# AnishDelft/ModelCompression

Measured on AMD Instinct MI355X. Metric: images/sec (fwd+bwd, 416x416), higher is better.
Workload: dtype fp16

## Files before the change

### include/mcamd.h

```cpp
#ifndef MCAMD_H
#define MCAMD_H

#include <stddef.h>
#include <stdint.h>

#ifdef __cplusplus
extern "C" {
#endif

#define MCAMD_OK 0
#define MCAMD_EINVAL (-1)
#define MCAMD_ELAUNCH (-2)
#define MCAMD_EWORKSPACE (-3)

int mcamd_version(void);
void mcamd_reload_config(void);
const char* mcamd_arch(void);
const char* mcamd_last_error(void);

typedef struct mcamd_conv_geom {
    int32_t B, H, W;
    int32_t ksize;
    int32_t cin;
    int32_t cout;
// ... 160 lines not shown
    int32_t ch_lo, C;
} mcamd_dgrad_sums;
int32_t mcamd_conv_dgrad_sums_rows(const mcamd_conv_geom* g, int32_t concurrent);
int mcamd_conv_dgrad_sums(const mcamd_conv_geom* g, const void* dy, int32_t dy_ld, int32_t dy_choff,
                          const void* wp_dgrad, const mcamd_conv_epilogue* epi, const mcamd_dgrad_sums* sums, void* stream);

size_t mcamd_conv_wgrad_workspace_bytes(const mcamd_conv_geom* g);
int mcamd_conv_wgrad(const mcamd_conv_geom* g, const void* x, const void* dy, int32_t dy_ld,
                     int32_t dy_choff, const float* mask_oihw, const mcamd_chan_map* map,
                     float grad_scale, float* dw_oihw, float* dbias, void* workspace,
                     size_t workspace_bytes, void* stream);

#define MCAMD_WGRAD_GENERIC 0
#define MCAMD_WGRAD_STEM 1
#define MCAMD_WGRAD_WIN 2
#define MCAMD_WGRAD_NINE 3
#define MCAMD_WGRAD_NINE_WIDE 4
#define MCAMD_WFIN_ROW 0
#define MCAMD_WFIN_VEC 1
#define MCAMD_WFIN_GENERIC 2
#define MCAMD_WGRAD_PLAN_INFO_N 13
int mcamd_conv_wgrad_plan_info(const mcamd_conv_geom* g, int32_t has_cmap, int32_t out[MCAMD_WGRAD_PLAN_INFO_N]);
int32_t mcamd_wgrad_generic_instances(int32_t* out, int32_t cap);

int mcamd_bn_coeffs(const float* stats, int32_t stats_rows, int32_t stats_ld, int32_t C, int64_t count,
                    const float* gamma, const float* beta, float* running_mean, float* running_var,
                    float momentum, float eps, int32_t training,
                    float* scale, float* shift, float* save_mean, float* save_invstd,
                    const int32_t* chan_perm, void* stream);

int mcamd_bn_coeffs_ex(const float* stats, int32_t stats_rows, int32_t stats_ld, int32_t C, int64_t count,
                       const float* gamma, const float* beta, float* running_mean, float* running_var,
                       float momentum, float eps, int32_t training,
                       float* scale, float* shift, float* save_mean, float* save_invstd,
                       const int32_t* chan_perm, int32_t ones_channel, void* stream);

#define MCAMD_DST_PLAIN 0
#define MCAMD_DST_POOL 1
#define MCAMD_DST_REORG 2
typedef struct mcamd_act_desc {
    int32_t B, H, W, C;
    const void* y; int32_t y_ld, y_choff;
    const float* scale; const float* shift;
    float slope;
    int32_t mode;
    void* dst; int32_t dst_ld, dst_choff;
// ... 328 lines not shown
```

### modelcompression_amd/_lib.py

```python
import ctypes as C
import os

_HERE = os.path.dirname(os.path.abspath(__file__))
LIB_PATH = os.path.join(_HERE, "libmcamd.so")


class McamdError(RuntimeError):
    pass


class ConvGeom(C.Structure):
    _fields_ = [("B", C.c_int32), ("H", C.c_int32), ("W", C.c_int32), ("ksize", C.c_int32),
                ("cin", C.c_int32), ("cout", C.c_int32), ("x_ld", C.c_int32), ("x_choff", C.c_int32),
                ("stem", C.c_int32), ("pad", C.c_int32), ("x_wrap", C.c_int32), ("x_f8", C.c_int32), ("x_f8_wexp", C.c_int32)]


class ConvEpilogue(C.Structure):
    _fields_ = [("mode", C.c_int32), ("y_ld", C.c_int32), ("y_choff", C.c_int32),
                ("y", C.c_void_p), ("bias", C.c_void_p), ("stats", C.c_void_p),
                ("stats_rows", C.c_int32), ("stats_ld", C.c_int32),
                ("scale", C.c_void_p), ("shift", C.c_void_p), ("slope", C.c_float), ("overflow", C.c_void_p),
                ("dst_mode", C.c_int32), ("y2", C.c_void_p), ("y2_ld", C.c_int32), ("y2_choff", C.c_int32),
                ("concurrent", C.c_int32)]

# ... 127 lines not shown


class WzSeg(C.Structure):
    _fields_ = [("w", C.c_void_p), ("mask", C.c_void_p), ("n", C.c_int64), ("word0", C.c_int64), ("val0", C.c_int64),
                ("kept", C.c_int64), ("cout", C.c_int32), ("kind", C.c_int32), ("exp0", C.c_int32), ("dense", C.c_int32),
                ("block0", C.c_int32), ("shift0", C.c_int32)]


class HzSeg(C.Structure):
    _fields_ = [("sym0", C.c_int64), ("nsym", C.c_int64), ("nbits", C.c_int64), ("word0", C.c_int64), ("chunk0", C.c_int64),
                ("popc_bits", C.c_int64), ("block0", C.c_int32), ("A", C.c_int32)]


class WsSeg(C.Structure):
    _fields_ = [("w", C.c_void_p), ("mask", C.c_void_p), ("codes", C.c_void_p), ("n", C.c_int64), ("part0", C.c_int64),
                ("K", C.c_int32), ("cb0", C.c_int32), ("slab0", C.c_int32), ("reserved", C.c_int32)]


EPI_RAW_F16, EPI_NCHW_F32, EPI_PAD_F16, EPI_RAW_F32 = 0, 1, 2, 3
DST_PLAIN, DST_POOL, DST_REORG = 0, 1, 2
WGRAD_GENERIC, WGRAD_STEM, WGRAD_WIN, WGRAD_NINE, WGRAD_NINE_WIDE = 0, 1, 2, 3, 4
WFIN_ROW, WFIN_VEC, WFIN_GENERIC = 0, 1, 2
WGRAD_PLAN_INFO_N = 13
STEM_PLAN_FWD, STEM_PLAN_FWD_PLANES, STEM_PLAN_STATS, STEM_PLAN_GRAM, STEM_PLAN_BWD = 0, 1, 2, 3, 4
STEM_PLAN_INFO_N = 20
WZ_FP32, WZ_FP16, WZ_FP8, WZ_CODE, WZ_W4 = 0, 1, 2, 4, 5
WZ_F_BN, WZ_F_BITS = 1, 2
WZ_BLOCK_WORDS = 64
HZ_MAXLEN, HZ_CHUNK, HZ_GROUP = 12, 1024, 64
WS_SLAB = 4096

_P, _I32, _I64, _F, _SZ = C.c_void_p, C.c_int32, C.c_int64, C.c_float, C.c_size_t
SIGNATURES = {
    "mcamd_version": (C.c_int, []),
    "mcamd_arch": (C.c_char_p, []),
    "mcamd_last_error": (C.c_char_p, []),
    "mcamd_reload_config": (None, []),
    "mcamd_conv_stats_rows": (_I32, [C.POINTER(ConvGeom)]),
    "mcamd_conv_stats_rows_mode": (_I32, [C.POINTER(ConvGeom), _I32]),
    "mcamd_conv_fwd_f8_ok": (_I32, [C.POINTER(ConvGeom)]),
    "mcamd_conv_tile_info": (C.c_int, [C.POINTER(ConvGeom), _I32, C.POINTER(_I32)]),
    "mcamd_conv_route_info": (C.c_int, [C.POINTER(ConvGeom), _I32, _I32, _I32, _I32, C.POINTER(_I32)]),
    "mcamd_packed_elems_fwd": (_I64, [C.POINTER(ConvGeom)]),
    "mcamd_packed_elems_dgrad": (_I64, [C.POINTER(ConvGeom)]),
    "mcamd_pack_weights": (C.c_int, [C.POINTER(ConvGeom), _P, _P, C.POINTER(ChanMap), _P, _P, _P]),
    "mcamd_pack_weights_many": (C.c_int, [_P, _I32, _I64, _P]),
# ... 28 lines not shown
    "mcamd_conv_fwd_q8_sparse24_ok": (_I32, [C.POINTER(ConvGeom)]),
    "mcamd_q8_sparse24_elems": (C.c_int, [C.POINTER(ConvGeom), C.POINTER(_I64)]),
    "mcamd_pack_q8_sparse24": (C.c_int, [C.POINTER(ConvGeom), _P, _P, _P, _P, _P, _P]),
    "mcamd_conv_fwd_q8_sparse24": (C.c_int, [C.POINTER(ConvGeom), _P, _P, _P, _P, C.POINTER(ConvEpilogue), _I32, _I32, _P]),
    "mcamd_conv_fwd_q8_w4_ok": (_I32, [C.POINTER(ConvGeom)]),
    "mcamd_q8_w4_elems": (C.c_int, [C.POINTER(ConvGeom), C.POINTER(_I64)]),
    "mcamd_pack_q8_w4": (C.c_int, [C.POINTER(ConvGeom), _P, _P, _P, _P, _P, _P]),
    "mcamd_unpack_q8_w4": (C.c_int, [C.POINTER(ConvGeom), _P, _P, _P, _P]),
    "mcamd_conv_fwd_q8_w4": (C.c_int, [C.POINTER(ConvGeom), _P, _P, _P, _P, C.POINTER(ConvEpilogue), _I32, _I32, _P]),
    "mcamd_conv_fwd_q8_w4_info": (C.c_int, [C.POINTER(ConvGeom), C.POINTER(_I32)]),
    "mcamd_conv_fwd_q8_w4_raw": (C.c_int, [C.POINTER(ConvGeom), _P, _P, _P, _P, C.POINTER(ConvEpilogue), _P]),
    "mcamd_fakequant_q8_w4": (C.c_int, [C.POINTER(ConvGeom), _P, _P, _P, _P, _P]),
    "mcamd_cast_q8": (C.c_int, [_P, _I64, _I32, _I32, _I32, _P, _I32, _I32, _P]),
    "mcamd_conv_fwd_q8_stats_rows": (_I32, [C.POINTER(ConvGeom)]),
    "mcamd_fakequant_q8": (C.c_int, [C.POINTER(ConvGeom), _P, _P, _P, _P, _P]),
    "mcamd_cast_q8_train": (C.c_int, [_P, _I64, _I32, _I32, _I32, _P, _I32, _I32, _P]),
    "mcamd_conv_dgrad": (C.c_int, [C.POINTER(ConvGeom), _P, _I32, _I32, _P, C.POINTER(ConvEpilogue), _P]),
    "mcamd_conv_dgrad_sums_rows": (_I32, [C.POINTER(ConvGeom), _I32]),
    "mcamd_conv_dgrad_sums": (C.c_int, [C.POINTER(ConvGeom), _P, _I32, _I32, _P, C.POINTER(ConvEpilogue), C.POINTER(DgradSums), _P]),
    "mcamd_conv_wgrad_workspace_bytes": (_SZ, [C.POINTER(ConvGeom)]),
    "mcamd_conv_wgrad": (C.c_int, [C.POINTER(ConvGeom), _P, _P, _I32, _I32, _P, C.POINTER(ChanMap), _F, _P, _P, _P, _SZ, _P]),
    "mcamd_conv_wgrad_plan_info": (C.c_int, [C.POINTER(ConvGeom), _I32, C.POINTER(_I32)]),
    "mcamd_wgrad_generic_instances": (_I32, [C.POINTER(_I32), _I32]),
    "mcamd_bn_coeffs": (C.c_int, [_P, _I32, _I32, _I32, _I64, _P, _P, _P, _P, _F, _F, _I32, _P, _P, _P, _P, _P, _P]),
    "mcamd_bn_coeffs_ex": (C.c_int, [_P, _I32, _I32, _I32, _I64, _P, _P, _P, _P, _F, _F, _I32, _P, _P, _P, _P, _P, _I32, _P]),
    "mcamd_fold_weights": (C.c_int, [C.POINTER(FoldDesc), _P, _P]),
    "mcamd_fold_weights_many": (C.c_int, [_P, _I32, _I64, _P]),
    "mcamd_unfold_wgrad": (C.c_int, [C.POINTER(FoldDesc), _P, _P, _P, _P, _I32, _P]),
    "mcamd_bn_act_fwd": (C.c_int, [C.POINTER(ActDesc), _P]),
    "mcamd_bn_act_fwd_instance": (C.c_int, [C.POINTER(ActDesc), C.POINTER(ActInstance)]),
    "mcamd_bn_act_conv1x1_ok": (_I32, [C.POINTER(ActDesc), C.POINTER(ConvGeom)]),
    "mcamd_bn_act_conv1x1_stats_rows": (_I32, [C.POINTER(ActDesc), C.POINTER(ConvGeom)]),
    "mcamd_bn_act_conv1x1_fwd": (C.c_int, [C.POINTER(ActDesc), C.POINTER(ConvGeom), _P, C.POINTER(ConvEpilogue), _P]),
    "mcamd_bn_act_bwd_workspace_bytes": (_SZ, [C.POINTER(ActBwdDesc)]),
    "mcamd_bn_act_bwd": (C.c_int, [C.POINTER(ActBwdDesc), _P, _SZ, _P]),
    "mcamd_stem_block_workspace_bytes": (_SZ, []),
    "mcamd_stem_block_fwd": (C.c_int, [C.POINTER(StemBlockDesc), _P, _SZ, _P]),
    "mcamd_stem_block_bwd": (C.c_int, [C.POINTER(StemBlockDesc), _P, _SZ, _P]),
    "mcamd_stem_block_stats_rows": (_I32, [C.POINTER(StemBlockDesc)]),
    "mcamd_stem_block_stats": (C.c_int, [C.POINTER(StemBlockDesc), _P, _I32, _I32, _P]),
    "mcamd_stem_block_plan_info": (C.c_int, [C.POINTER(StemBlockDesc), C.POINTER(_I32)]),
    "mcamd_nchw_f32_to_nhwc4_split": (C.c_int, [_P, _I32, _I32, _I32, _P, _P, _P]),
    "mcamd_pack_stem_split": (C.c_int, [_P, _P, _I32, _P, _P, _P]),
    "mcamd_nchw_f32_to_padded_nhwc_f16": (C.c_int, [_P, _I32, _I32, _I32, _I32, _F, _P, _I32, _I32, _P, _P]),
    "mcamd_nchw_f32_to_padded_nhwc_f16_pad": (C.c_int, [_P, _I32, _I32, _I32, _I32, _F, _P, _I32, _I32, _I32, _P, _P]),
    "mcamd_nchw_f32_to_padded_nhwc_f16_split": (C.c_int, [_P, _I32, _I32, _I32, _I32, _P, _I32, _I32, _I32, _P]),
# ... 91 lines not shown
```

### modelcompression_amd/build.py

```python
import os
import subprocess
import sys
from concurrent.futures import ThreadPoolExecutor

HERE = os.path.dirname(os.path.abspath(__file__))
CSRC = os.path.join(HERE, "csrc")
OUT = os.path.join(HERE, "libmcamd.so")
HIPCC = os.environ.get("HIPCC", "/opt/rocm/bin/hipcc")
ARCH = "gfx950"
COMMON = ["--offload-arch=" + ARCH, "-O3", "-fPIC", "-std=c++17", "-Wall", "-Wno-unused-variable",
          "-fhip-fp32-correctly-rounded-divide-sqrt"]
SOURCES = {
    "api.hip": [],
    "conv_igemm.hip": [],
    "conv_igemm_pp.hip": [],
    "conv_sparse.hip": [],
    "conv_bsparse.hip": [],
    "conv_splitk.hip": [],
    "conv_q8.hip": [],
    "conv_q8_sparse.hip": [],
    "conv_q8_splitk.hip": [],
    "conv_q8_bsparse.hip": [],
    "conv_q8_w4.hip": [],
    "conv_stem.hip": [],
    "conv_stem_block.hip": [],
    "conv_stem_f32.hip": [],
    "conv_small.hip": [],
    "conv_win.hip": [],
    "conv_wres.hip": [],
    "conv_wgrad.hip": [],
    "conv_wgrad_stem.hip": [],
    "bn_act.hip": [],
    "bn_conv1x1.hip": [],
    "fold.hip": [],
    "plan.hip": [],
    "region_loss.hip": [],
    "distill_loss.hip": [],
    "prune.hip": ["-ffp-contract=off"],
    "augment.hip": ["-ffp-contract=off"],
    "detect.hip": ["-ffp-contract=off"],
    "voc_eval.hip": ["-ffp-contract=off"],
    "wpack.hip": ["-ffp-contract=off"],
    "wshare.hip": ["-ffp-contract=off"],
    "huff.hip": [],
}


def _stale(target, deps):
    if not os.path.exists(target):
        return True
    t = os.path.getmtime(target)
    return any(os.path.getmtime(d) > t for d in deps)


# ... 33 lines not shown
```

### modelcompression_amd/csrc/api.hip

```cpp
#include <stdarg.h>
#include <stdlib.h>
#include <string.h>

#include <string>

#include "kernels.h"

static thread_local char g_err[512] = "";

void mcamd_set_error(const char* fmt, ...) {
    va_list ap;
    va_start(ap, fmt);
    vsnprintf(g_err, sizeof(g_err), fmt, ap);
    va_end(ap);
}

int g_mcamd_env_generation = 0;
int McamdEnvSlot::get(const char* name, int dflt) {
    const int g = __atomic_load_n(&g_mcamd_env_generation, __ATOMIC_ACQUIRE);
    if (gen != g) {
        const char* s = getenv(name);
        has = s && *s ? 1 : 0;
        val = has ? atoi(s) : 0;
        __atomic_store_n(&gen, g, __ATOMIC_RELEASE);
// ... 1284 lines not shown
    a.dy_off = dy_choff + a.dy_row_stride + dy_ld;
    a.dy_zero_off = dy_choff;
    a.H = g->H, a.W = g->W, a.HW = g->H * g->W;
    a.M = (int)M;
    a.cin_tap = cin_tap;
    a.ntaps = ntaps;
    a.ktot = ntaps * cin_tap;
    fill_taps(g->ksize, g->stem, a.x_row_stride, g->x_ld, a.tap_off);
    int rc = p.nine    ? mcamd_wgrad9_launch(a, p, g->W + pw_of(g), padded_pixels(g), st)
             : p.stemw == 1 ? mcamd_wgrad_stem_launch(a, p, st)
             : p.stemw == 2 ? mcamd_wgrad_win_launch(a, p, st)
                       : mcamd_wgrad_launch(a, p, st);
    if (rc) return rc;
    rc = mcamd_wgrad_finish_launch((const float*)workspace, p, a.ktot, cin_tap, g->stem, g->cout, g->cin, g->ksize,
                                   mask_oihw, 1.0f / grad_scale, dw_oihw, rmap, cmap, st);
    if (rc) return rc;
    if (dbias) {
        long long rows = padded_pixels(g);
        rc = mcamd_colsum_launch((const half_t*)dy, rows, dy_ld, dy_choff, g->cout, 1.0f / grad_scale, dbias, st, workspace,
                                 workspace_bytes);
    }
    return rc;
}
```

### modelcompression_amd/csrc/kernels.h

```cpp
#pragma once
#include "common.h"

struct DgradSums {
    float* slab;
    const half_t* act;
    const float* scale;
    const float* shift;
    const float* mean;
    const float* invstd;
    const float* y;
    int act_ld, act_choff, act_pw;
    int y_ld, y_choff;
    int ch_lo, C;
    int ld;
    float slope;
};
#define MCAMD_EPI_RAW_F16_SUMS 4

struct IgemmArgs {
    const half_t* x;
    const half_t* w;
    void* y;
    const float* bias;
    float* stats;
// ... 121 lines not shown
int mcamd_pack_q8_sparse24_launch(const float* w, const float* mask, void* wq, void* idx, void* wexp, int cout, int cin,
                                  int ntaps, hipStream_t st);
Q8Choice mcamd_q8_w4_choice(long long M, int N);
int mcamd_conv_q8_w4_launch(IgemmArgs& a, const void* gshift, const void* wexp, int y_f8, int y2_f8, hipStream_t st);
int mcamd_pack_q8_w4_launch(const float* w, const float* mask, void* codes, void* gshift, void* wexp, int cout, int cin, int ntaps,
                            hipStream_t st);
int mcamd_unpack_q8_w4_launch(const void* codes, const void* gshift, void* wq, int cout, int cin, int ntaps, hipStream_t st);
int mcamd_conv_q8_w4_raw_launch(IgemmArgs& a, const void* gshift, const void* wexp, hipStream_t st);
int mcamd_fakequant_q8_w4_launch(const void* codes, const void* gshift, const void* wexp, float* out, int cout, int cin, int ntaps,
                                 hipStream_t st);

WgradPlan mcamd_wgrad_plan(long long M, int cout, int cin_tap, int ntaps);
int mcamd_wgrad_launch(WgradArgs& a, const WgradPlan& p, hipStream_t st);
bool mcamd_wgrad_stem_ok(int stem, int cout, int W, long long M);
WgradPlan mcamd_wgrad_stem_plan(long long M);
int mcamd_wgrad_stem_launch(WgradArgs& a, const WgradPlan& p, hipStream_t st);
bool mcamd_wgrad_win_ok(int ksize, int stem, int cout, int cin_tap, int W, long long M);
WgradPlan mcamd_wgrad_win_plan(long long M, int cout);
int mcamd_wgrad_win_launch(WgradArgs& a, const WgradPlan& p, hipStream_t st);
bool mcamd_wgrad_use9(int ksize, int stem, int cout, int cin_tap, int W);
WgradPlan mcamd_wgrad_plan9(long long P, int cout, int cin_tap, int W, int pitch, int B);
int mcamd_wgrad9_launch(const WgradArgs& w, const WgradPlan& p, int pitch, long long P, hipStream_t st);
WgradFinish mcamd_wgrad_finish_pick(int nsplit, int stem, int Cin, int ksize, bool has_cmap);
int mcamd_wgrad_instances(int (*out)[4], int cap);
int mcamd_wgrad_finish_launch(const float* slab, const WgradPlan& p, int ktot, int cin_tap, int stem, int Cout, int Cin,
                              int ksize, const float* mask, float inv_scale, float* dw, const int* rmap, const int* cmap,
                              hipStream_t st);
int mcamd_colsum_launch(const half_t* dy, long long rows, int ld, int choff, int C, float inv_scale, float* out,
                        hipStream_t st, void* scratch, size_t scratch_bytes);

bool mcamd_win3x3_ok(int mode, bool stats, long long M, int n, int cin_tap, int ktot, int H, int W);
int mcamd_win3x3_launch(const IgemmArgs& a, hipStream_t st);
bool mcamd_small3x3_ok(long long M, int n, int cin_tap, int ktot);
int mcamd_small3x3_rows(long long M);
int mcamd_small3x3_launch(const IgemmArgs& a, int rows, hipStream_t st);
bool mcamd_small3x3_split_ok(long long M, int n, int cin_tap, int ktot, int wrap, int mode);
int mcamd_small3x3_split_launch(const IgemmArgs& a, int rows, hipStream_t st);

bool mcamd_bn_conv1x1_shape_ok(int P, int cout);
int mcamd_bn_conv1x1_launch(IgemmArgs& a, const float* py, int py_ld, int py_choff, int P, int rows, hipStream_t st);

bool mcamd_wres_ok(int ksize, int stem, int n, int cin_tap, int ktot, int B, int H, int W, int mode);
int mcamd_wres_rows(int n, int B, int H, int W);
int mcamd_wres_launch(IgemmArgs& a, int B, int rows, hipStream_t st);

bool mcamd_stem_direct_ok(int stem, int cout, int mode);
// ... 3 lines not shown
```

### modelcompression_amd/engine.py

```python
import contextlib
import math
import os
import time

import torch

from . import ops
from . import _lib as L
from ._lib import McamdError


class _T:
    __slots__ = ("buf", "ld", "choff", "C", "H", "W", "ps", "ps0")

    def __init__(self, buf, ld, choff, C, H, W, ps=0):
        self.buf, self.ld, self.choff, self.C, self.H, self.W, self.ps = buf, ld, choff, C, H, W, ps
        self.ps0 = ps


_LAYER_FIELDS = dict(
    index=0, li=0, conv=None, bn=None, slope=1.0, src=0, tin=None, cin=0, cout=0, cout_p=0, H=0, W=0, k=0, M=0, stem=0, pad=0,
    level=1, mode=0, out_id=None, out2_id=None, out_t=None, out2_t=None, is_last=False, train_ok=True, border=None,
    border_map=None, geom=None, geom_f=None, p_lo=0, p_hi=0,
    wp=None, wd=None, y=None, stats=None, scale=None, shift=None, mean=None, invstd=None, dy=None, gin=None, act_full=None,
    keep=None, perm=None, perm32=None, in_perm=None, g_rows=None, g_cols=None, n_act=0, geom_act=None, gather=False,
    fold=None, fold_cin=0, fold_aug=0, fold_consumers=None, ones_idx=-1, skip_dead=False, bn_width=0, waug=None, dwaug=None,
    fused_stem=False, fused_stem_eval=False, stem_shadow=False, stem_split=False, stem_f32=False, stem_ws=None, weff=None,
    sh_img=None, sh_img_lo=None, sh_geom=None, sh_wp=None, sh_wp_lo=None, sh_coef=None,
    f8=False, f8_wexp=ops.F8_WEXP_DEFAULT, f8_wexp_eff=ops.F8_WEXP_DEFAULT,
    form="dense", sk_slices=1, wsp=None, widx=None, bs_count=None, bs_list=None,
    geom_q8=None, q8_y=False, q8_y2=False, xq=None, _xq=None, _xq_key=None, wq=None, wqs=None, widx8=None, wexp=None,
    w4c=None, w4g=None, wexp4=None,
    y_f16=None, stats_f16=None, y_f32=None, stats_q8=None, w_q=None)


class _Layer:
    __slots__ = tuple(_LAYER_FIELDS)

    def __init__(self):
        for name, default in _LAYER_FIELDS.items():
            setattr(self, name, default)
        self.fold_consumers = []

    sp_on = property(lambda self: self.form == "sparse24")
    bs_on = property(lambda self: self.form == "bsparse")
    sk_on = property(lambda self: self.form == "splitk")
# ... 516 lines not shown
                budget = int((MIXED_BUDGET / PLAIN_BLOCK_ERR) ** 2)
                unsplittable = len(self.layers) - len(can) - (1 if self.stem else 0)
                plain = set(l.li for l in by_cost[:max(0, budget - unsplittable)])
            for lay in can:
                if lay.li not in plain:
                    lay.level = 3
        f32 = dict(dtype=torch.float32, device=dev)
        wbytes = 0

        def li_is_first(l):
            return l.li == 0
        for lay in self.layers:
            g = lay.geom
            wrap = 2 * lay.tin.ps if (self.act_planes == 2 and lay.li > 0) else 0
            lay.geom_f = g if lay.level == 1 else ops.geom(B, lay.H, lay.W, lay.k, lay.level * lay.cin, lay.cout,
                                                           lay.tin.ld, 0, 0, lay.pad, wrap)
            nf, _ = ops.packed_elems(lay.geom_f)
            if self.precise:
                lay.n_act, lay.geom_act = lay.cout, g
                self._set_geom_f(lay)
            _, nd = ops.packed_elems(g)
            lay.wp = torch.zeros(nf, dtype=ops.HALF, device=dev)
            lay.wd = torch.zeros(nd, dtype=ops.HALF, device=dev) if (nd and lay.li > 0) else None
            wbytes = max(wbytes, ops.wgrad_workspace_bytes(g))
            lay.cout_p = ops.round_up(lay.cout, 32)
            lay.fused_stem = bool(lay.stem and lay.bn is not None and lay.mode == L.DST_POOL and lay.out2_id is None
                                  and lay.cout == 32 and lay.W % 32 == 0 and lay.H % 2 == 0 and lay.border is None)
            lay.fused_stem_eval = bool(lay.stem and lay.bn is not None and lay.mode == L.DST_POOL and lay.out2_id is None
                                       and lay.cout in (8, 16, 24) and lay.W % 32 == 0 and lay.H % 2 == 0 and lay.border is None)
            lay.stem_shadow = bool(li_is_first(lay) and self.stem_shadow and lay.bn is not None and lay.mode == L.DST_POOL
                                   and lay.out2_id is None and lay.cout == 32 and lay.border is None)
            lay.stem_split = lay.stem_shadow
            if lay.stem_shadow:
                lay.sh_img = ops.alloc_padded(B, lay.H, lay.W, 4, dev)
                lay.sh_geom = ops.geom(B, lay.H, lay.W, 3, 3, lay.cout, 4, 0, 1)
                lay.sh_wp = torch.zeros(ops.packed_elems(lay.sh_geom)[0], dtype=ops.HALF, device=dev)
                lay.sh_img_lo = ops.alloc_padded(B, lay.H, lay.W, 4, dev)
                lay.sh_wp_lo = torch.zeros_like(lay.sh_wp)
                lay.sh_coef = [torch.empty(lay.cout, **f32) for _ in range(4)]
                lay.stem_ws = torch.empty(ops.stem_block_workspace_bytes(), dtype=torch.uint8, device=dev)
            lay.dy = None if (lay.fused_stem or lay.stem_shadow) else ops.alloc_padded(B, lay.H, lay.W, lay.cout_p, dev, pad=lay.pad)
            if lay.li > 0:
                lay.gin = torch.empty(lay.M * lay.tin.ld, dtype=ops.HALF, device=dev)
            lay.n_act, lay.geom_act = lay.cout, lay.geom
            if not lay.is_last:
                if lay.fused_stem:
                    lay.stem_ws = torch.empty(ops.stem_block_workspace_bytes(), dtype=torch.uint8, device=dev)
# ... 1007 lines not shown
                if lay.out2_id is not None and lay.out2_id in self.consumer_of:
                    c2, t2 = self.consumer_of[lay.out2_id], lay.out2_t
                    g2, g2_ld, g2_choff = c2.gin, c2.tin.ld, t2.choff
                self.bn_act_bwd_layer(lay, cons.gin, cons.tin.ld, t.choff, g2, g2_ld or 0, g2_choff or 0, lay.dy,
                                      gmap[id(lay.bn.weight)], gmap[id(lay.bn.bias)], D, sums=sums_of.pop(lay.li, None))
            mask = lay.conv.mask.contiguous() if lay.conv.mask_flag else None
            dbias = gmap[id(lay.conv.bias)] if lay.conv.bias is not None else None
            def wgrad_of(ws, lay=lay, mask=mask, dbias=dbias):
                if lay.fold is not None:
                    gw, prod = gmap[id(lay.conv.weight)], lay.fold
                    if lay.perm is not None:
                        ops.memset_zero(gw)
                    self._timed('wgrad', lay, ops.conv_wgrad, lay.geom_act, self.bufs[lay.tin.buf], lay.dy, lay.cout_p, 0,
                                lay.dwaug, None, D, dbias, ws)
                    ops.unfold_wgrad(lay.conv.weight.data, mask, lay.g_rows, lay.g_cols, prod.bn.bias.data, prod.slope, lay.n_act,
                                     lay.fold_cin, lay.dwaug, gw, gmap[id(prod.bn.bias)], gmap[id(prod.bn.weight)],
                                     accumulate=prod.fold_consumers[0] is not lay)
                elif lay.gather:
                    gw = gmap[id(lay.conv.weight)]
                    if lay.perm is not None:
                        ops.memset_zero(gw)
                    self._timed('wgrad', lay, ops.conv_wgrad, lay.geom_act, self.bufs[lay.tin.buf], lay.dy, lay.cout_p, 0,
                                gw, mask, D, dbias, ws, rows=lay.g_rows, cols=lay.g_cols)
                else:
                    self._timed('wgrad', lay, ops.conv_wgrad, lay.geom, self.bufs[lay.tin.buf], lay.dy, lay.cout_p, 0,
                                gmap[id(lay.conv.weight)], mask, D, dbias, ws)

            if side is None:
                wgrad_of(self.wgrad_ws)
                ready(lay)
            else:
                pending.append((wgrad_of, lay))
                if len(pending) >= chunk or lay.li <= 1:
                    flush()
            if lay.li > 0:
                conc = side is not None and self._side_concurrent
                ds = self._dgrad_sums(lay, conc)
                if ds is not None:
                    sums_of[ds[2].li] = ds[1]
                self._timed('dgrad', lay, ops.conv_dgrad_raw, lay.geom_act, lay.dy, lay.cout_p, 0, lay.wd, lay.gin, lay.tin.ld,
                            lay.tin.choff, overflow=self.overflow, concurrent=conc, sums=ds[0] if ds is not None else None)
        if side is not None:
            flush()
            ops.stream_wait(main, side)
```

### modelcompression_amd/ops.py

```python
import collections
import ctypes as C
import weakref

import torch

from . import _lib as L
from ._lib import (ConvGeom, ConvEpilogue, SplitkInfo, ActDesc, ActBwdDesc, DgradSums, ChanMap, PackJob, StemBlockDesc, FoldDesc, FoldJob, check, ptr,
                   stream_ptr)

HALF = torch.float16
SLACK = 64


def round_up(v, m):
    return (v + m - 1) // m * m


def _need_cuda(*ts):
    for t in ts:
        if t is not None and not t.is_cuda:
            raise L.McamdError("modelcompression_amd compute ops need CUDA (MI355X) tensors; there is no CPU path")


def guard_elems(W, ld):
# ... 205 lines not shown

WgradPlanInfo = collections.namedtuple("WgradPlanInfo", "family tmo tnc taps kp ns nsplit pix_per_split rows_pad finish sg tiles grid")


def wgrad_plan_info(g, has_cmap=False):
    out = (C.c_int32 * L.WGRAD_PLAN_INFO_N)()
    check(L.lib().mcamd_conv_wgrad_plan_info(C.byref(g), 1 if has_cmap else 0, out), "mcamd_conv_wgrad_plan_info")
    return WgradPlanInfo(*out)


def wgrad_generic_instances():
    lib = L.lib()
    n = int(lib.mcamd_wgrad_generic_instances(None, 0))
    out = (C.c_int32 * (4 * n))()
    lib.mcamd_wgrad_generic_instances(out, n)
    return [tuple(out[4 * i:4 * i + 4]) for i in range(n)]


def conv_wgrad(g, x, dy, dy_ld, dy_choff, dw, mask=None, grad_scale=1.0, dbias=None, workspace=None, rows=None, cols=None):
    if workspace is None:
        workspace = torch.empty(wgrad_workspace_bytes(g), dtype=torch.uint8, device=dw.device)
    check(L.lib().mcamd_conv_wgrad(C.byref(g), ptr(x), ptr(dy), dy_ld, dy_choff, ptr(mask), _chan_map(g, rows, cols), grad_scale, ptr(dw),
                                   ptr(dbias), ptr(workspace), workspace.numel(), stream_ptr()), "mcamd_conv_wgrad")


def _perm_ptr(perm, C_):
    if perm is None:
        return None
    if perm.dtype != torch.int32 or perm.numel() != C_ or not perm.is_contiguous() or not perm.is_cuda:
        raise L.McamdError("channel permutation must be a contiguous CUDA int32 vector of %d entries" % C_)
    return perm.data_ptr()


def bn_coeffs(stats, C_, count, gamma, beta, rmean, rvar, training, scale, shift, mean=None, invstd=None,
              momentum=0.1, eps=1e-5, perm=None, ones_channel=-1):
    rows = stats.shape[0] if stats is not None else 0
    ld = stats.shape[2] if stats is not None else 0
    check(L.lib().mcamd_bn_coeffs_ex(ptr(stats), rows, ld, C_, count, ptr(gamma), ptr(beta), ptr(rmean), ptr(rvar),
                                     momentum, eps, 1 if training else 0, ptr(scale), ptr(shift), ptr(mean), ptr(invstd),
                                     _perm_ptr(perm, C_), ones_channel, stream_ptr()), "mcamd_bn_coeffs_ex")


def _fold_desc(w, mask, rows, cols, beta, slope, n, cin_k, aug):
    _need_cuda(w, mask, rows, cols, beta)
    assert w.dtype == torch.float32 and w.is_contiguous() and w.dim() == 4 and w.shape[2] == w.shape[3]
    assert beta.dtype == torch.float32 and beta.numel() == w.shape[1]
# ... 1264 lines not shown
```

Before: 5786.

## Add dedicated 1x1 weight-gradient GEMM kernel with split-K and LDS pipelining

Adds a specialised weight-gradient kernel for dense 1x1 convolutions. It treats wgrad as a dy^T·x GEMM over pixels, using 32x32x16 MFMA, a 3-stage direct global-to-LDS pipeline with swizzled transposed reads, and split-K over pixels written to a float slab that the existing finish kernel reduces. The engine routes eligible 1x1 layers to this path by default, with an environment variable to turn it off. It adds another workspace-size requirement and a new kernel whose tiling may not beat the generic path for every shape.

Result: no change. 5825 (median of 6 runs) (+0.7%).

```diff
diff --git a/include/mcamd.h b/include/mcamd.h
--- a/include/mcamd.h
+++ b/include/mcamd.h
@@ -206,6 +206,13 @@
 #define MCAMD_WGRAD_PLAN_INFO_N 13
 int mcamd_conv_wgrad_plan_info(const mcamd_conv_geom* g, int32_t has_cmap, int32_t out[MCAMD_WGRAD_PLAN_INFO_N]);
 int32_t mcamd_wgrad_generic_instances(int32_t* out, int32_t cap);
+
+#define MCAMD_WGRAD_1X1_PLAN_INFO_N 12
+size_t mcamd_conv_wgrad_1x1_workspace_bytes(const mcamd_conv_geom* g);
+int mcamd_conv_wgrad_1x1_plan_info(const mcamd_conv_geom* g, int32_t has_cmap, int32_t out[MCAMD_WGRAD_1X1_PLAN_INFO_N]);
+int mcamd_conv_wgrad_1x1(const mcamd_conv_geom* g, const void* x, const void* dy, int32_t dy_ld, int32_t dy_choff,
+                         const float* mask_oihw, float grad_scale, float* dw_oihw, float* dbias, void* workspace,
+                         size_t workspace_bytes, void* stream);
 
 int mcamd_bn_coeffs(const float* stats, int32_t stats_rows, int32_t stats_ld, int32_t C, int64_t count,
                     const float* gamma, const float* beta, float* running_mean, float* running_var,
diff --git a/modelcompression_amd/_lib.py b/modelcompression_amd/_lib.py
--- a/modelcompression_amd/_lib.py
+++ b/modelcompression_amd/_lib.py
@@ -173,6 +173,7 @@
 WGRAD_GENERIC, WGRAD_STEM, WGRAD_WIN, WGRAD_NINE, WGRAD_NINE_WIDE = 0, 1, 2, 3, 4
 WFIN_ROW, WFIN_VEC, WFIN_GENERIC = 0, 1, 2
 WGRAD_PLAN_INFO_N = 13
+WGRAD_1X1_PLAN_INFO_N = 12
 STEM_PLAN_FWD, STEM_PLAN_FWD_PLANES, STEM_PLAN_STATS, STEM_PLAN_GRAM, STEM_PLAN_BWD = 0, 1, 2, 3, 4
 STEM_PLAN_INFO_N = 20
 WZ_FP32, WZ_FP16, WZ_FP8, WZ_CODE, WZ_W4 = 0, 1, 2, 4, 5
@@ -247,6 +248,9 @@
     "mcamd_conv_wgrad": (C.c_int, [C.POINTER(ConvGeom), _P, _P, _I32, _I32, _P, C.POINTER(ChanMap), _F, _P, _P, _P, _SZ, _P]),
     "mcamd_conv_wgrad_plan_info": (C.c_int, [C.POINTER(ConvGeom), _I32, C.POINTER(_I32)]),
     "mcamd_wgrad_generic_instances": (_I32, [C.POINTER(_I32), _I32]),
+    "mcamd_conv_wgrad_1x1_workspace_bytes": (_SZ, [C.POINTER(ConvGeom)]),
+    "mcamd_conv_wgrad_1x1": (C.c_int, [C.POINTER(ConvGeom), _P, _P, _I32, _I32, _P, _F, _P, _P, _P, _SZ, _P]),
+    "mcamd_conv_wgrad_1x1_plan_info": (C.c_int, [C.POINTER(ConvGeom), _I32, C.POINTER(_I32)]),
     "mcamd_bn_coeffs": (C.c_int, [_P, _I32, _I32, _I32, _I64, _P, _P, _P, _P, _F, _F, _I32, _P, _P, _P, _P, _P, _P]),
     "mcamd_bn_coeffs_ex": (C.c_int, [_P, _I32, _I32, _I32, _I64, _P, _P, _P, _P, _F, _F, _I32, _P, _P, _P, _P, _P, _I32, _P]),
     "mcamd_fold_weights": (C.c_int, [C.POINTER(FoldDesc), _P, _P]),
diff --git a/modelcompression_amd/build.py b/modelcompression_amd/build.py
--- a/modelcompression_amd/build.py
+++ b/modelcompression_amd/build.py
@@ -30,6 +30,7 @@
     "conv_wres.hip": [],
     "conv_wgrad.hip": [],
     "conv_wgrad_stem.hip": [],
+    "conv_wgrad_1x1.hip": [],
     "bn_act.hip": [],
     "bn_conv1x1.hip": [],
     "fold.hip": [],
diff --git a/modelcompression_amd/csrc/api.hip b/modelcompression_amd/csrc/api.hip
--- a/modelcompression_amd/csrc/api.hip
+++ b/modelcompression_amd/csrc/api.hip
@@ -1330,3 +1330,68 @@
     }
     return rc;
 }
+
+static bool wgrad_1x1_eligible(const mcamd_conv_geom* g) { return mcamd_wgrad1x1_ok(g->ksize, g->stem, g->cin, padded_pixels(g)); }
+
+static size_t wgrad_1x1_bytes(const mcamd_conv_geom* g, const WgradPlan& p) {
+    const size_t colsum = (size_t)128 * round_up_int(g->cout, 8) * sizeof(float);
+    return p.bytes > colsum ? p.bytes : colsum;
+}
+
+extern "C" size_t mcamd_conv_wgrad_1x1_workspace_bytes(const mcamd_conv_geom* g) {
+    if (!g || !wgrad_1x1_eligible(g)) return 0;
+    return wgrad_1x1_bytes(g, mcamd_wgrad1x1_plan(padded_pixels(g), g->cout, cin_tap_of(g)));
+}
+
+extern "C" int mcamd_conv_wgrad_1x1_plan_info(const mcamd_conv_geom* g, int32_t has_cmap, int32_t out[MCAMD_WGRAD_1X1_PLAN_INFO_N]) {
+    if (check_geom(g, "conv_wgrad_1x1_plan_info")) return MCAMD_EINVAL;
+    MCAMD_REQUIRE(out, "conv_wgrad_1x1_plan_info: null output");
+    memset(out, 0, sizeof(int32_t) * MCAMD_WGRAD_1X1_PLAN_INFO_N);
+    if (has_cmap || !wgrad_1x1_eligible(g)) return MCAMD_OK;
+    const WgradPlan p = mcamd_wgrad1x1_plan(padded_pixels(g), g->cout, cin_tap_of(g));
+    const WgradFinish f = mcamd_wgrad_finish_pick(p.nsplit, 0, g->cin, 1, false);
+    const int tiles = p.n_otiles * p.n_ctiles;
+    out[0] = 1;
+    out[1] = p.tmo, out[2] = p.tnc, out[3] = p.kp, out[4] = p.ns;
+    out[5] = p.nsplit, out[6] = p.pix_per_split, out[7] = p.rows_pad;
+    out[8] = tiles;
+    out[9] = f.kernel, out[10] = f.sg;
+    out[11] = round_up_int(tiles * p.nsplit, 8);
+    return MCAMD_OK;
+}
+
+extern "C" int mcamd_conv_wgrad_1x1(const mcamd_conv_geom* g, const void* x, const void* dy, int32_t dy_ld, int32_t dy_choff,
+                                    const float* mask_oihw, float grad_scale, float* dw_oihw, float* dbias, void* workspace,
+                                    size_t workspace_bytes, void* stream) {
+    if (mcamd_recording()) {
+        MCAMD_REQUIRE(g, "conv_wgrad_1x1: null geometry");
+        const mcamd_conv_geom g_ = *g;
+        return mcamd_rec_push(stream, [=](void* s) {
+            return mcamd_conv_wgrad_1x1(&g_, x, dy, dy_ld, dy_choff, mask_oihw, grad_scale, dw_oihw, dbias, workspace, workspace_bytes, s);
+        });
+    }
+    if (check_geom(g, "conv_wgrad_1x1")) return MCAMD_EINVAL;
+    MCAMD_REQUIRE(g->x_wrap == 0 && g->x_f8 == 0, "conv_wgrad_1x1: x_wrap / x_f8 are forward-only fields");
+    MCAMD_REQUIRE(wgrad_1x1_eligible(g), "conv_wgrad_1x1: not a dense 1x1 layer with cin %% 4 == 0 (ksize %d, stem %d, cin %d): use mcamd_conv_wgrad", g->ksize, g->stem, g->cin);
+    MCAMD_REQUIRE(x && dy && dw_oihw && workspace, "conv_wgrad_1x1: null argument");
+    MCAMD_REQUIRE(grad_scale > 0.f, "conv_wgrad_1x1: grad_scale must be positive");
+    const int cin_tap = cin_tap_of(g);
+    const long long P = padded_pixels(g);
+    const WgradPlan p = mcamd_wgrad1x1_plan(P, g->cout, cin_tap);
+    MCAMD_REQUIRE(dy_ld % 8 == 0 && dy_choff % 8 == 0 && dy_choff >= 0 && dy_choff + p.rows_pad <= dy_ld,
+                  "conv_wgrad_1x1: dy slice [%d, %d) does not fit dy_ld %d", dy_choff, dy_choff + p.rows_pad, dy_ld);
+    if (workspace_bytes < p.bytes) {
+        mcamd_set_error("conv_wgrad_1x1: workspace %zu < %zu bytes", workspace_bytes, p.bytes);
+        return MCAMD_EWORKSPACE;
+    }
+    hipStream_t st = (hipStream_t)stream;
+    int rc = mcamd_wgrad1x1_launch((const half_t*)x + g->x_choff, g->x_ld, (const half_t*)dy + dy_choff, dy_ld, P, cin_tap,
+                                   (float*)workspace, p, st);
+    if (rc) return rc;
+    rc = mcamd_wgrad_finish_launch((const float*)workspace, p, cin_tap, cin_tap, 0, g->cout, g->cin, 1, mask_oihw,
+                                   1.0f / grad_scale, dw_oihw, nullptr, nullptr, st);
+    if (rc) return rc;
+    if (dbias)
+        rc = mcamd_colsum_launch((const half_t*)dy, P, dy_ld, dy_choff, g->cout, 1.0f / grad_scale, dbias, st, workspace, workspace_bytes);
+    return rc;
+}
diff --git a/modelcompression_amd/csrc/conv_wgrad_1x1.hip b/modelcompression_amd/csrc/conv_wgrad_1x1.hip
--- /dev/null
+++ b/modelcompression_amd/csrc/conv_wgrad_1x1.hip
@@ -0,0 +1,236 @@
+#include "kernels.h"
+#include "tr_frag.h"
+#include <string.h>
+
+struct Wgrad1Args {
+    const half_t* x;
+    const half_t* dy;
+    float* slab;
+    int x_ld, dy_ld;
+    int cin_tap;
+    int rows_pad;
+    int P;
+    int n_otiles, n_ctiles, nsplit, pix_per_split;
+};
+
+template <int RB>
+__device__ __forceinline__ unsigned w1_lane_off(int colbase, int lane) {
+    const int g = lane >> 4, i16 = lane & 15, q = i16 >> 2, p = i16 & 3;
+    const int row = 8 * (g >> 1) + q;
+    const int off = (colbase + 16 * (g & 1) + 4 * p) * 2;
+    return row * RB + ((((off >> 4) ^ tr_swz<RB>(row)) << 4) | (off & 15));
+}
+
+template <int S_, int RBA, int RBB, int FM, int FN>
+__device__ __forceinline__ void w1_issue(unsigned sa, unsigned sb, const unsigned (&a_lo)[FM], const unsigned (&b_lo)[FN],
+                                         Frag (&af)[FM], Frag (&bf)[FN]) {
+#pragma unroll
+    for (int i = 0; i < FM; ++i) {
+        af[i].lo = tr_read4<S_ * 16 * RBA>(sa + a_lo[i]);
+        af[i].hi = tr_read4<S_ * 16 * RBA + 4 * RBA>(sa + a_lo[i]);
+    }
+#pragma unroll
+    for (int j = 0; j < FN; ++j) {
+        bf[j].lo = tr_read4<S_ * 16 * RBB>(sb + b_lo[j]);
+        bf[j].hi = tr_read4<S_ * 16 * RBB + 4 * RBB>(sb + b_lo[j]);
+    }
+}
+
+template <int FM, int FN>
+__device__ __forceinline__ void w1_mfma(Frag (&af)[FM], Frag (&bf)[FN], f32x16_t (&acc)[FM][FN]) {
+#pragma unroll
+    for (int i = 0; i < FM; ++i) tie(af[i]);
+#pragma unroll
+    for (int j = 0; j < FN; ++j) tie(bf[j]);
+#pragma unroll
+    for (int i = 0; i < FM; ++i)
+#pragma unroll
+        for (int j = 0; j < FN; ++j)
+            acc[i][j] = __builtin_amdgcn_mfma_f32_32x32x16_f16(af[i].v(), bf[j].v(), acc[i][j], 0, 0, 0);
+}
+
+template <int TM, int TN, int KP, int NS>
+__global__ __launch_bounds__(256) void wgrad1x1_kernel(Wgrad1Args a) {
+    constexpr int NT = 256;
+    constexpr int RBA = TM * 2, RBB = TN * 2;
+    constexpr int A_CH = TM / 8, B_CH = TN / 8;
+    constexpr int A_IT = KP * A_CH / NT, B_IT = KP * B_CH / NT;
+    constexpr int A_BYTES = KP * RBA, STAGE_BYTES = KP * (RBA + RBB);
+    constexpr int FM = TM / 64, FN = TN / 64;
+    constexpr int CNT = A_IT + B_IT;
+    static_assert((KP * A_CH) % NT == 0 && (KP * B_CH) % NT == 0, "every thread issues every DMA instruction");
+    static_assert(KP == 64, "the stage is written out for four k16 sub-steps");
+    static_assert(NS == 3, "the counted wait below knows one younger stage");
+
+    extern __shared__ __attribute__((aligned(16))) char smem[];
+    const int tid = threadIdx.x, lane = tid & 63;
+    const int wave = __builtin_amdgcn_readfirstlane(tid >> 6);
+    const int wm = wave >> 1, wn = wave & 1;
+    const unsigned smem_addr = lds_addr_of(smem);
+
+    const int ntiles = a.n_otiles * a.n_ctiles;
+    const int total_items = ntiles * a.nsplit;
+    const int chunk = (total_items + 7) >> 3;
+    const int item = (blockIdx.x & 7) * chunk + (blockIdx.x >> 3);
+    if ((int)(blockIdx.x >> 3) >= chunk || item >= total_items) return;
+    const int split = item / ntiles;
+    const int tile = item - split * ntiles;
+    const int ot = tile / a.n_ctiles, ct = tile - ot * a.n_ctiles;
+    const int k0 = split * a.pix_per_split;
+    int k1 = k0 + a.pix_per_split;
+    if (k1 > a.P) k1 = a.P;
+    const int nsteps = k1 > k0 ? (k1 - k0 + KP - 1) / KP : 0;
+
+    int a_col[A_IT], b_col[B_IT];
+#pragma unroll
+    for (int it = 0; it < A_IT; ++it) {
+        const int slot = it * NT + tid, row = slot / A_CH;
+        int col = ot * TM + (((slot % A_CH) ^ tr_swz<RBA>(row)) * 8);
+        a_col[it] = col < a.rows_pad ? col : 0;
+    }
+#pragma unroll
+    for (int it = 0; it < B_IT; ++it) {
+        const int slot = it * NT + tid, row = slot / B_CH;
+        int col = ct * TN + (((slot % B_CH) ^ tr_swz<RBB>(row)) * 8);
+        b_col[it] = col < a.cin_tap ? col : 0;
+    }
+
+    auto stage = [&](int p0, int buf) {
+        char* sa = smem + buf * STAGE_BYTES;
+        char* sb = sa + A_BYTES;
+        const bool tail = p0 + KP > a.P;
+#pragma unroll
+        for (int it = 0; it < A_IT; ++it) {
+            long long prow = p0 + (it * NT + tid) / A_CH;
+            if (tail && prow >= a.P) prow = 0;
+            glds16(a.dy + prow * a.dy_ld + a_col[it], sa + (it * NT + wave * 64) * 16);
+        }
+#pragma unroll
+        for (int it = 0; it < B_IT; ++it) {
+            long long prow = p0 + (it * NT + tid) / B_CH;
+            if (tail && prow >= a.P) prow = 0;
+            glds16(a.x + prow * a.x_ld + b_col[it], sb + (it * NT + wave * 64) * 16);
+        }
+    };
+
+    f32x16_t acc[FM][FN];
+#pragma unroll
+    for (int i = 0; i < FM; ++i)
+#pragma unroll
+        for (int j = 0; j < FN; ++j)
+#pragma unroll
+            for (int r = 0; r < 16; ++r) acc[i][j][r] = 0.f;
+
+    unsigned a_lo[FM], b_lo[FN];
+#pragma unroll
+    for (int i = 0; i < FM; ++i) a_lo[i] = w1_lane_off<RBA>(wm * (TM / 2) + i * 32, lane);
+#pragma unroll
+    for (int j = 0; j < FN; ++j) b_lo[j] = w1_lane_off<RBB>(wn * (TN / 2) + j * 32, lane);
+
+#pragma unroll
+    for (int k = 0; k < NS - 1; ++k)
+        if (k < nsteps) stage(k0 + k * KP, k);
+    int slot = 0;
+    for (int st = 0; st < nsteps; ++st) {
+        if (st + 1 < nsteps) wait_vmcnt<CNT>();
+        else wait_vmcnt<0>();
+        __syncthreads();
+        if (st + NS - 1 < nsteps) {
+            int nslot = slot + NS - 1;
+            if (nslot >= NS) nslot -= NS;
+            stage(k0 + (st + NS - 1) * KP, nslot);
+        }
+        const unsigned sa = smem_addr + slot * STAGE_BYTES;
+        const unsigned sb = sa + A_BYTES;
+        slot = slot + 1 == NS ? 0 : slot + 1;
+        Frag af0[FM], bf0[FN], af1[FM], bf1[FN];
+        w1_issue<0, RBA, RBB, FM, FN>(sa, sb, a_lo, b_lo, af0, bf0);
+        lds_wait_all(af0[0]);
+        w1_issue<1, RBA, RBB, FM, FN>(sa, sb, a_lo, b_lo, af1, bf1);
+        w1_mfma<FM, FN>(af0, bf0, acc);
+        lds_wait_all(af1[0]);
+        w1_issue<2, RBA, RBB, FM, FN>(sa, sb, a_lo, b_lo, af0, bf0);
+        w1_mfma<FM, FN>(af1, bf1, acc);
+        lds_wait_all(af0[0]);
+        w1_issue<3, RBA, RBB, FM, FN>(sa, sb, a_lo, b_lo, af1, bf1);
+        w1_mfma<FM, FN>(af0, bf0, acc);
+        lds_wait_all(af1[0]);
+        w1_mfma<FM, FN>(af1, bf1, acc);
+    }
+
+    float* out = a.slab + (long long)split * a.rows_pad * a.cin_tap;
+#pragma unroll
+    for (int i = 0; i < FM; ++i)
+#pragma unroll
+        for (int j = 0; j < FN; ++j) {
+            const int k = ct * TN + wn * (TN / 2) + j * 32 + (lane & 31);
+#pragma unroll
+            for (int r = 0; r < 16; ++r) {
+                const int n = ot * TM + wm * (TM / 2) + i * 32 + mfma32_row(r, lane);
+                if (n < a.rows_pad && k < a.cin_tap) out[(long long)n * a.cin_tap + k] = acc[i][j][r];
+            }
+        }
+}
+
+#define MCAMD_W1_KP 64
+#define MCAMD_W1_NS 3
+#define MCAMD_W1_MIN_STEPS 8
+
+bool mcamd_wgrad1x1_ok(int ksize, int stem, int cin, long long P) {
+    return ksize == 1 && !stem && cin % 4 == 0 && P > 0 && P < (1ll << 31) - MCAMD_W1_KP;
+}
+
+WgradPlan mcamd_wgrad1x1_plan(long long P, int cout, int cin_tap) {
+    WgradPlan p;
+    memset(&p, 0, sizeof(p));
+    p.rows_pad = round_up_int(cout, 32);
+    p.tmo = p.rows_pad <= 64 ? 64 : 128;
+    p.tnc = 128;
+    p.taps = 1;
+    p.kp = MCAMD_W1_KP;
+    p.ns = MCAMD_W1_NS;
+    p.n_otiles = (p.rows_pad + p.tmo - 1) / p.tmo;
+    p.n_ctiles = (cin_tap + p.tnc - 1) / p.tnc;
+    p.n_tapgroups = 1;
+    const long long tiles = (long long)p.n_otiles * p.n_ctiles;
+    const long long resident = p.tmo == 128 ? 256 : 512;
+    const long long steps = (P + p.kp - 1) / p.kp;
+    long long ns = resident / tiles;
+    if (ns > steps / MCAMD_W1_MIN_STEPS) ns = steps / MCAMD_W1_MIN_STEPS;
+    if (ns < 1) ns = 1;
+    const long long sps = (steps + ns - 1) / ns;
+    ns = (steps + sps - 1) / sps;
+    p.nsplit = (int)ns;
+    p.pix_per_split = (int)(sps * p.kp);
+    p.bytes = (size_t)p.nsplit * p.rows_pad * (size_t)cin_tap * sizeof(float);
+    return p;
+}
+
+template <int TM>
+static void launch_w1(const Wgrad1Args& a, int grid, hipStream_t st) {
+    constexpr size_t lds = (size_t)MCAMD_W1_NS * MCAMD_W1_KP * (TM + 128) * 2;
+    MCAMD_LDS_OPT_IN((wgrad1x1_kernel<TM, 128, MCAMD_W1_KP, MCAMD_W1_NS>), lds);
+    hipLaunchKernelGGL((wgrad1x1_kernel<TM, 128, MCAMD_W1_KP, MCAMD_W1_NS>), dim3(grid), dim3(256), lds, st, a);
+}
+
+int mcamd_wgrad1x1_launch(const half_t* x, int x_ld, const half_t* dy, int dy_ld, long long P, int cin_tap, float* slab,
+                          const WgradPlan& p, hipStream_t st) {
+    Wgrad1Args a;
+    memset(&a, 0, sizeof(a));
+    a.x = x, a.dy = dy, a.slab = slab;
+    a.x_ld = x_ld, a.dy_ld = dy_ld;
+    a.cin_tap = cin_tap;
+    a.rows_pad = p.rows_pad;
+    a.P = (int)P;
+    a.n_otiles = p.n_otiles, a.n_ctiles = p.n_ctiles;
+    a.nsplit = p.nsplit, a.pix_per_split = p.pix_per_split;
+    const int grid = round_up_int(p.n_otiles * p.n_ctiles * p.nsplit, 8);
+    if (p.tnc == 128 && p.kp == MCAMD_W1_KP && p.ns == MCAMD_W1_NS && p.tmo == 128) launch_w1<128>(a, grid, st);
+    else if (p.tnc == 128 && p.kp == MCAMD_W1_KP && p.ns == MCAMD_W1_NS && p.tmo == 64) launch_w1<64>(a, grid, st);
+    else {
+        mcamd_set_error("wgrad_1x1: no kernel instance for tile %dx%d kp %d stages %d", p.tmo, p.tnc, p.kp, p.ns);
+        return MCAMD_EINVAL;
+    }
+    MCAMD_LAUNCH_CHECK("wgrad_1x1");
+    return MCAMD_OK;
+}
diff --git a/modelcompression_amd/csrc/kernels.h b/modelcompression_amd/csrc/kernels.h
--- a/modelcompression_amd/csrc/kernels.h
+++ b/modelcompression_amd/csrc/kernels.h
@@ -167,6 +167,10 @@
 WgradPlan mcamd_wgrad_plan9(long long P, int cout, int cin_tap, int W, int pitch, int B);
 int mcamd_wgrad9_launch(const WgradArgs& w, const WgradPlan& p, int pitch, long long P, hipStream_t st);
 WgradFinish mcamd_wgrad_finish_pick(int nsplit, int stem, int Cin, int ksize, bool has_cmap);
+bool mcamd_wgrad1x1_ok(int ksize, int stem, int cin, long long P);
+WgradPlan mcamd_wgrad1x1_plan(long long P, int cout, int cin_tap);
+int mcamd_wgrad1x1_launch(const half_t* x, int x_ld, const half_t* dy, int dy_ld, long long P, int cin_tap, float* slab,
+                          const WgradPlan& p, hipStream_t st);
 int mcamd_wgrad_instances(int (*out)[4], int cap);
 int mcamd_wgrad_finish_launch(const float* slab, const WgradPlan& p, int ktot, int cin_tap, int stem, int Cout, int Cin,
                               int ksize, const float* mask, float inv_scale, float* dw, const int* rmap, const int* cmap,
diff --git a/modelcompression_amd/engine.py b/modelcompression_amd/engine.py
--- a/modelcompression_amd/engine.py
+++ b/modelcompression_amd/engine.py
@@ -21,7 +21,7 @@
 _LAYER_FIELDS = dict(
     index=0, li=0, conv=None, bn=None, slope=1.0, src=0, tin=None, cin=0, cout=0, cout_p=0, H=0, W=0, k=0, M=0, stem=0, pad=0,
     level=1, mode=0, out_id=None, out2_id=None, out_t=None, out2_t=None, is_last=False, train_ok=True, border=None,
-    border_map=None, geom=None, geom_f=None, p_lo=0, p_hi=0,
+    border_map=None, geom=None, geom_f=None, p_lo=0, p_hi=0, wgrad_1x1_ok=False,
     wp=None, wd=None, y=None, stats=None, scale=None, shift=None, mean=None, invstd=None, dy=None, gin=None, act_full=None,
     keep=None, perm=None, perm32=None, in_perm=None, g_rows=None, g_cols=None, n_act=0, geom_act=None, gather=False,
     fold=None, fold_cin=0, fold_aug=0, fold_consumers=None, ones_idx=-1, skip_dead=False, bn_width=0, waug=None, dwaug=None,
@@ -584,7 +584,9 @@
             _, nd = ops.packed_elems(g)
             lay.wp = torch.zeros(nf, dtype=ops.HALF, device=dev)
             lay.wd = torch.zeros(nd, dtype=ops.HALF, device=dev) if (nd and lay.li > 0) else None
-            wbytes = max(wbytes, ops.wgrad_workspace_bytes(g))
+            wbytes = max(wbytes, ops.wgrad_workspace_bytes(g), ops.wgrad_1x1_workspace_bytes(lay.geom))
+            lay.wgrad_1x1_ok = (lay.k == 1 and os.environ.get("MCAMD_WGRAD_1X1", "1") == "1"
+                                and bool(ops.wgrad_1x1_plan_info(lay.geom).eligible))
             lay.cout_p = ops.round_up(lay.cout, 32)
             lay.fused_stem = bool(lay.stem and lay.bn is not None and lay.mode == L.DST_POOL and lay.out2_id is None
                                   and lay.cout == 32 and lay.W % 32 == 0 and lay.H % 2 == 0 and lay.border is None)
@@ -1638,6 +1640,9 @@
                         ops.memset_zero(gw)
                     self._timed('wgrad', lay, ops.conv_wgrad, lay.geom_act, self.bufs[lay.tin.buf], lay.dy, lay.cout_p, 0,
                                 gw, mask, D, dbias, ws, rows=lay.g_rows, cols=lay.g_cols)
+                elif lay.wgrad_1x1_ok:
+                    self._timed('wgrad', lay, ops.conv_wgrad_1x1, lay.geom, self.bufs[lay.tin.buf], lay.dy, lay.cout_p, 0,
+                                gmap[id(lay.conv.weight)], mask, D, dbias, ws)
                 else:
                     self._timed('wgrad', lay, ops.conv_wgrad, lay.geom, self.bufs[lay.tin.buf], lay.dy, lay.cout_p, 0,
                                 gmap[id(lay.conv.weight)], mask, D, dbias, ws)
diff --git a/modelcompression_amd/ops.py b/modelcompression_amd/ops.py
--- a/modelcompression_amd/ops.py
+++ b/modelcompression_amd/ops.py
@@ -251,6 +251,26 @@
         workspace = torch.empty(wgrad_workspace_bytes(g), dtype=torch.uint8, device=dw.device)
     check(L.lib().mcamd_conv_wgrad(C.byref(g), ptr(x), ptr(dy), dy_ld, dy_choff, ptr(mask), _chan_map(g, rows, cols), grad_scale, ptr(dw),
                                    ptr(dbias), ptr(workspace), workspace.numel(), stream_ptr()), "mcamd_conv_wgrad")
+
+
+def wgrad_1x1_workspace_bytes(g):
+    return int(L.lib().mcamd_conv_wgrad_1x1_workspace_bytes(C.byref(g)))
+
+
+Wgrad1x1PlanInfo = collections.namedtuple("Wgrad1x1PlanInfo", "eligible tm tn kp ns nsplit pix_per_split rows_pad tiles finish sg grid")
+
+
+def wgrad_1x1_plan_info(g, has_cmap=False):
+    out = (C.c_int32 * L.WGRAD_1X1_PLAN_INFO_N)()
+    check(L.lib().mcamd_conv_wgrad_1x1_plan_info(C.byref(g), 1 if has_cmap else 0, out), "mcamd_conv_wgrad_1x1_plan_info")
+    return Wgrad1x1PlanInfo(*out)
+
+
+def conv_wgrad_1x1(g, x, dy, dy_ld, dy_choff, dw, mask=None, grad_scale=1.0, dbias=None, workspace=None):
+    if workspace is None:
+        workspace = torch.empty(wgrad_1x1_workspace_bytes(g), dtype=torch.uint8, device=dw.device)
+    check(L.lib().mcamd_conv_wgrad_1x1(C.byref(g), ptr(x), ptr(dy), dy_ld, dy_choff, ptr(mask), grad_scale, ptr(dw), ptr(dbias),
+                                       ptr(workspace), workspace.numel(), stream_ptr()), "mcamd_conv_wgrad_1x1")
 
 
 def _perm_ptr(perm, C_):
```
